# BerserkerMother/Video-Summarization

Measured on AMD Instinct MI355X. Metric: frames/sec scored (whole node), synthetic [B,T=1024,D=1024], higher is better.
Workload: dtype f32; 1 GPU; configs[2]: B=64 videos x T=1024 frames x D=1024 per GPU, scorer cfg M-A (heads 4, d_model 256, layers 4), logits + hidden state; global_batch=64, parallelism=videos sharded over 1 GPU(s), no all_gather of scores

## Files before the change

### video-summarization_amd/csrc/vs_kernels.h

```cpp
#pragma once
#include <hip/hip_runtime.h>
#include <stdint.h>

enum { VSK_STORE16 = 16, VSK_A16 = 32, VSK_F16 = 64 };
int vsk_linear(const float *A, const float *W, const float *Wf, const float *bias, float *C, int M, int N, int K,
               int relu, const float *pe, int T, int bf16, hipStream_t st);
int vsk_linear_gate(const float *A, const float *W, const float *Wf, const float *bias, const float *gate, float scale,
                    float *C, int M, int N, int K, hipStream_t st, int bf16 = 0);
int vsk_linear_relu_dropout(const float *A, const float *W, const float *Wf, const float *bias, float *C, int M, int N,
                            int K, unsigned long long seed, unsigned site, float p, hipStream_t st, int bf16 = 0);
int vsk_pack_fragments(const float *W, float *Wf, int N, int K, hipStream_t st);
int vsk_pack_fragments_f16x3(const float *W, float *Wh, int N, int K, hipStream_t st);
int vsk_qkv(const float *h, const float *Wqkv, const float *Wf, const float *bqkv, float *qkv, int B, int T, int d,
            int H, int bf16, hipStream_t st, float qscale = 1.0f);
int vsk_attention(const float *q, const float *k, const float *v, const uint8_t *mask, float *out,
                  int B, int H, int T, int dh, float scale, hipStream_t st);
int vsk_attention_packed(const float *q, const float *k, const float *v, float *out, int H, int Mtot, int dh,
                         float scale, const int *cu, const int *work, int nwork, int nw, int prec, hipStream_t st);
float vsk_attention_qscale(float scale);
int vsk_attention_bf16(const float *q, const float *k, const float *v, const uint8_t *mask, float *out,
                       int B, int H, int T, int dh, float scale, int prec, hipStream_t st);
int vsk_attention_bf16_w64(const void *q, const void *k, const void *v, const uint8_t *mask, void *out, int B, int H, int T,
                           hipStream_t st);
int vsk_attention_bf16_w64_packed(const void *q, const void *k, const void *v, void *out, int H, int Mtot, const int *cu,
                                  const int *work, int nwork, hipStream_t st);
size_t vsk_attention_probs_workspace_bytes(int B, int H, int T);
int vsk_attention_probs(const float *q, const float *k, const uint8_t *mask, float *maps, float *received, float *entropy,
                        int B, int H, int T, int dh, float scale, void *workspace, hipStream_t st);
int vsk_linear_res_ln(const float *A, const float *W, const float *Wf, const float *bias, const float *res,
                      const float *gamma, const float *beta, float *out, int M, int N, int K,
                      const float *score_w, const float *score_b, int num_classes, int sigmoid,
                      float *scores, int bf16, hipStream_t st);
int vsk_rows_res_ln(const float *a, const float *res, const float *gamma, const float *beta, float *out, int M, int d,
                    const float *score_w, const float *score_b, int num_classes, int sigmoid, float *scores,
                    hipStream_t st, void *out16 = nullptr, int dn = 0,
                    int nsplit = 0, const float *pbias = nullptr);
struct VskMatJobs {
    enum { MAX = 24 };
    const float *in[MAX];
    float *out[MAX];
    int rows[MAX], cols[MAX];
    int n;
};
int vsk_pack_fragments_batch(const VskMatJobs &jobs, hipStream_t st);
int vsk_attention_splitkv(const float *q, const float *k, const float *v, const uint8_t *mask, float *out,
                          int B, int H, int T, int dh, float scale, hipStream_t st);
int vsk_linear_parts(const float *A, const float *Wf, float *parts, int M, int N, int K, int nsplit, hipStream_t st,
                     int f16x3 = 0);
int vsk_sum_parts_pe(const float *parts, int nsplit, const float *bias, const float *pe, int T, float *out, int M, int N, hipStream_t st);
int vsk_diag_attention(const float *q, const float *k, const float *v, float *out, int B, int H, int T, float scale,
                       unsigned long long *diag, hipStream_t st);
int vsk_diag_attention_lp(const float *q, const float *k, const float *v, float *out, int B, int H, int T, float scale,
                          int prec, unsigned long long *diag, hipStream_t st);
int vsk_diag_gemm(const float *A, const float *W, const float *bias, float *C, int M, int N, int K,
                  int grid, unsigned long long *diag, hipStream_t st);
int vsk_mlp_fused(const float *H1, const float *W1, const float *b1, const float *W2, const float *b2,
                  const float *gamma, const float *beta, float *out, int M, int d,
                  const float *score_w, const float *score_b, int num_classes, int sigmoid, float *scores,
                  hipStream_t st);
bool vsk_mlp_bf16_supported(int d);
size_t vsk_mlp_bf16_image_bytes(int d);
int vsk_pack_mlp_bf16(const float *Wo, const float *W1, const float *W2, void *img, int d, hipStream_t st);
struct VskNextQkv {
    const void *img;
    const float *bqkv;
// ... 12 lines not shown
                 const float *gamma, const float *beta, float *out, int M, int d,
                 const float *score_w, const float *score_b, int num_classes, int sigmoid, float *scores,
                 const VskNextQkv *next, hipStream_t st);
int vsk_plan_packed(const int *lengths_dev, int B, int qb, int *cu, int *work, int work_cap, hipStream_t st);
int vsk_gather_rows(const float *pe, const int *cu, int B, int tmax, int d, float *rows, hipStream_t st);
enum { VSK_COPY_MAX_SEGS = 20 };
struct VskCopySegs {
    const float *src[VSK_COPY_MAX_SEGS];
    float *dst[VSK_COPY_MAX_SEGS];
    unsigned n[VSK_COPY_MAX_SEGS];
    int count;
};
int vsk_copy_segments(const VskCopySegs &segs, hipStream_t st);
int vsk_insert_cls(const float *e, const float *cls, const uint8_t *mask, float *h, uint8_t *mask1, int B, int T, int d,
                   hipStream_t st);
int vsk_skinny_max_rows();

struct VskOptions {
    int skinny_rows;
    int lp_min_rows;
    int train_lp_min_rows;
    int lp_min_rows_fused;
    int gemm_nwm2;
    int gemm_nj2;
    int attn_nw4;
    int attn_lp_simple;
    int attn_w64;
    int lp_store32;
    int lp_mlp_unfused;
    int lp_tail_unfused;
    int lp_qkv_unfused;
    int lp_tile256;
    int lp_embed_unfused;
    int mlp_fusion;
    int mlp_abl;
    int attn_w64_checked;
    int attn_legacy;
    int attn_w64_abl;
};
VskOptions &vsk_options();
int vsk_device_cus();

bool vsk_gemm16_supported(int M, int N, int K);
int vsk_gemm16(const void *A16, const void *W16, const float *bias, void *C, int M, int N, int K, int epi, int c16,
               int T, int H, int dh, float qscale, hipStream_t st);
int vsk_to_bf16(const float *src, void *dst, size_t n, hipStream_t st);
```

### video-summarization_amd/csrc/vs_kernels.hip

```cpp
#include <atomic>

#include "vs_train_device.h"
#include "vs_kernels.h"

namespace {

enum { EPI_BIAS = 0, EPI_RELU = 1, EPI_PE = 2, EPI_QKV = 3,
       EPI_GATE = 4,
       EPI_RELU_DROP = 5 };
struct EpiArgs {
    unsigned long long seed;
    unsigned site;
    float p;
    float scale;
};

__device__ __forceinline__ unsigned long long stamp() { return vs_stamp(); }

template <int EPI, int NWM = 2, int DIAG = 0, int NJ = 2, int PREC = 0, int C16 = 0, int KW = 32, int A16 = 0>
__global__ __launch_bounds__(128 * NWM, 2) void gemm_nt_128(
    const float *__restrict__ A, const float *__restrict__ W, const float *__restrict__ bias,
    float *__restrict__ C, int M, int N, int K, const float *__restrict__ pe, int T, int H, int dh,
    unsigned long long *__restrict__ diag = nullptr, EpiArgs ea = EpiArgs{0ull, 0u, 0.f, 0.f}) {
    static_assert(KW == 32 || (KW == 64 && (PREC == 1 || PREC == 3)), "64-wide k-tiles exist for the 16-bit operands only");
// ... 516 lines not shown
            if (row < M) out[(size_t)row * N + cbase + 32 * j] = y;
        }
    }
    if (score_w != nullptr) {
        for (int c = 0; c < num_classes; ++c) {
            __syncthreads();
            float wj[NB];
#pragma unroll
            for (int j = 0; j < NB; ++j) wj[j] = score_w[(size_t)c * N + cbase + 32 * j];
#pragma unroll
            for (int t = 0; t < 16; ++t) {
                float s = 0.f;
#pragma unroll
                for (int j = 0; j < NB; ++j) s += acc[j][t] * wj[j];
                part[t] = half_sum(s);
            }
            if (r == 0) {
#pragma unroll
                for (int t = 0; t < 16; ++t) red[wc * 64 + 32 * wr + acc_row(t, h)] = part[t];
            }
            __syncthreads();
            if (tid < 64) {
                const int row = m0 + tid;
                if (row < M) {
                    float s = red[tid] + red[64 + tid] + score_b[c];
                    if (sigmoid) s = 1.0f / (1.0f + expf(-s));
                    scores[(size_t)row * num_classes + c] = s;
                }
            }
        }
    }
}

template <int NT, int PREC = 0, int A16 = 0, int DIAG = 0>
__global__ __launch_bounds__(256, 2) void gemm_ln_rows(
    const float *__restrict__ A, const float *__restrict__ W, const float *__restrict__ bias,
    const float *__restrict__ res, const float *__restrict__ gamma, const float *__restrict__ beta,
    float *__restrict__ out, int M, int K,
    const float *__restrict__ score_w, const float *__restrict__ score_b, int num_classes,
    int sigmoid, float *__restrict__ scores, unsigned long long *__restrict__ diag = nullptr) {
    constexpr int BM = 128, N = 32 * NT, BK = 16, LD = BK + 4;
    constexpr int WL = (N * BK / 4 + 255) / 256;
    __shared__ __attribute__((aligned(16))) float smem[2 * (BM + N) * LD + 4 * N];
    float *gam_s = smem + 2 * (BM + N) * LD, *bet_s = gam_s + N, *sw_s = bet_s + N, *bias_s = sw_s + N;

    const int tid = threadIdx.x, lane = tid & 63, wave = tid >> 6;
    const int r = lane & 31, h = lane >> 5;
    const int ntiles = (M + BM - 1) / BM;
    const int nk = K / BK;

    constexpr float SC = PREC == 2 ? F16X3_WS : 1.0f;
    for (int i = tid; i < N; i += 256) { gam_s[i] = gamma[i]; bet_s[i] = beta[i]; bias_s[i] = bias[i] * SC; }

    const int lrow = tid >> 2, lc4 = (tid & 3) * 4;
    f32x4 pa[2], pw[WL];
    u32x2 pa16[2];
    const float *aptr[2], *wptr[WL];
    const unsigned short *aptr16[2];
#pragma unroll
    for (int i = 0; i < WL; ++i) {
        int wrow = lrow + 64 * i; wrow = wrow < N ? wrow : N - 1;
        wptr[i] = W + (size_t)wrow * K + lc4;
    }
    static_assert(PREC != 0 || N % 64 == 0, "the exact-fp32 staging map covers W without a guard");
    __amdgpu_buffer_rsrc_t ars = __builtin_amdgcn_make_buffer_rsrc(const_cast<float *>(A), 0, 0, 0x00020000);
    const __amdgpu_buffer_rsrc_t wrs = __builtin_amdgcn_make_buffer_rsrc(const_cast<float *>(W), 0, N * K * 4, 0x00020000);
    int aoff[2], woff[WL];
#pragma unroll
    for (int i = 0; i < WL; ++i) woff[i] = ((lrow + 64 * i) * K + lc4) * 4;
    auto gload = [&](int i, int kb) __attribute__((always_inline)) {
        if (i < 2) pa[i] = __builtin_bit_cast(f32x4, __builtin_amdgcn_raw_buffer_load_b128(ars, aoff[i], kb, 0));
        else pw[i - 2] = __builtin_bit_cast(f32x4, __builtin_amdgcn_raw_buffer_load_b128(wrs, woff[i - 2], kb, 0));
    };
    constexpr int LDB = 12;
    auto stage = [&](int buf) __attribute__((always_inline)) {
        float *As = smem + buf * (BM + N) * LD, *Ws = As + BM * LD;
        if constexpr (PREC == 2) {
#pragma unroll
            for (int i = 0; i < 2; ++i) {
                u32x2 hi, lo;
                split_f16x4((const float *)&pa[i], hi, lo);
                *(u32x2 *)&As[(lrow + 64 * i) * LD + lc4 / 2] = hi;
                *(u32x2 *)&As[(lrow + 64 * i) * LD + 8 + lc4 / 2] = lo;
            }
#pragma unroll
            for (int i = 0; i < WL; ++i)
                if (lrow + 64 * i < N) {
                    u32x2 hi, lo;
                    const f32x4 ws = pw[i] * F16X3_WS;
                    split_f16x4((const float *)&ws, hi, lo);
                    *(u32x2 *)&Ws[(lrow + 64 * i) * LD + lc4 / 2] = hi;
                    *(u32x2 *)&Ws[(lrow + 64 * i) * LD + 8 + lc4 / 2] = lo;
                }
        } else if constexpr (PREC == 1) {
#pragma unroll
            for (int i = 0; i < 2; ++i) {
                u32x2 u;
                if constexpr (A16 != 0) u = pa16[i];
                else { u[0] = pack_bf16(pa[i][0], pa[i][1]); u[1] = pack_bf16(pa[i][2], pa[i][3]); }
                *(u32x2 *)&As[(lrow + 64 * i) * LDB + lc4 / 2] = u;
            }
#pragma unroll
            for (int i = 0; i < WL; ++i)
                if (lrow + 64 * i < N) {
                    u32x2 u; u[0] = pack_bf16(pw[i][0], pw[i][1]); u[1] = pack_bf16(pw[i][2], pw[i][3]);
                    *(u32x2 *)&Ws[(lrow + 64 * i) * LDB + lc4 / 2] = u;
                }
        } else {
#pragma unroll
            for (int i = 0; i < 2; ++i) *(f32x4 *)&As[(lrow + 64 * i) * LD + lc4] = pa[i];
#pragma unroll
            for (int i = 0; i < WL; ++i) *(f32x4 *)&Ws[(lrow + 64 * i) * LD + lc4] = pw[i];
        }
    };

    f32x16 acc[NT];
    unsigned long long dsum[3] = {0, 0, 0}, tbegin = 0, tq = 0, ktiles = 0;
    if constexpr (DIAG != 0) tbegin = stamp();
    for (int tile = blockIdx.x; tile < ntiles; tile += gridDim.x) {
        if constexpr (DIAG != 0) tq = stamp();
        const int m0 = tile * BM;
        int row = m0 + 32 * wave + r;
        const bool row_ok = row < M;
        row = row_ok ? row : M - 1;
#pragma unroll
        for (int i = 0; i < 2; ++i) {
            int ar = m0 + lrow + 64 * i; ar = ar < M ? ar : M - 1;
            if constexpr (A16 != 0) {
                aptr16[i] = (const unsigned short *)A + (size_t)ar * K + lc4;
                pa16[i] = *(const u32x2 *)aptr16[i];
            } else if constexpr (PREC == 0) {
                aoff[i] = ((ar - m0) * K + lc4) * 4;
            } else {
                aptr[i] = A + (size_t)ar * K + lc4;
                pa[i] = *(const f32x4 *)aptr[i];
            }
        }
        if constexpr (PREC == 0) {
            ars = __builtin_amdgcn_make_buffer_rsrc(const_cast<float *>(A + (size_t)m0 * K), 0, (M - m0 < BM ? M - m0 : BM) * K * 4, 0x00020000);
#pragma unroll
            for (int i = 0; i < 2 + WL; ++i) gload(i, 0);
        } else {
#pragma unroll
            for (int i = 0; i < WL; ++i) pw[i] = *(const f32x4 *)wptr[i];
        }
        {
            const float *rp = res + (size_t)row * N + 4 * h;
#pragma unroll
            for (int j = 0; j < NT; ++j)
// ... 71 lines not shown
                int nld = 0, nwr = 0;
#pragma unroll
                for (int q = 0; q < LPS; ++q) {
                    const int il = t * LPS + q, iw = (t - WB) * LPS + q;
                    if (il < NL) { gload(il, kn * (BK * 4)); ++nld; }
                    if (t >= WB && iw < NL) {
                        float *Ad = smem + ((kt + 1) & 1) * (BM + N) * LD, *Wd = Ad + BM * LD;
                        if (iw < 2) *(f32x4 *)&Ad[(lrow + 64 * iw) * LD + lc4] = pa[iw];
                        else *(f32x4 *)&Wd[(lrow + 64 * (iw - 2)) * LD + lc4] = pw[iw - 2];
                        ++nwr;
                    }
                }
#pragma unroll
                for (int s2 = 0; s2 < 4; ++s2) acc[j] = MFMA32(fw[t % 3][s2], fa[g][s2], acc[j]);
                __builtin_amdgcn_sched_group_barrier(0x008, 1, 0);
                if (t + 2 < NS) __builtin_amdgcn_sched_group_barrier(0x100, 1, 0);
#pragma unroll
                for (int q = 0; q < LPS; ++q)
                    if (q < nld) __builtin_amdgcn_sched_group_barrier(0x020, 1, 0);
                __builtin_amdgcn_sched_group_barrier(0x008, 3, 0);
#pragma unroll
                for (int q = 0; q < LPS; ++q)
                    if (q < nwr) __builtin_amdgcn_sched_group_barrier(0x200, 1, 0);
                __builtin_amdgcn_sched_barrier(0);
            }
            if constexpr (DIAG != 0) {
                const unsigned long long tb = stamp();
                __syncthreads();
                dsum[0] += stamp() - tb;
            } else
                __syncthreads();
        }
        if constexpr (DIAG != 0) tq = stamp();

        float sum = 0.f;
#pragma unroll
        for (int j = 0; j < NT; ++j) {
            float pj = 0.f;
#pragma unroll
            for (int q = 0; q < 4; ++q) {
                const f32x4 bv = *(const f32x4 *)&bias_s[32 * j + 8 * q + 4 * h];
#pragma unroll
                for (int e = 0; e < 4; ++e) { acc[j][4 * q + e] += bv[e]; pj += acc[j][4 * q + e]; }
            }
            sum += pj;
        }
        sum = pair_sum(sum);
        const float mean = sum * (1.0f / N);
        float sq = 0.f;
#pragma unroll
        for (int j = 0; j < NT; ++j) {
            float pj = 0.f;
#pragma unroll
            for (int t = 0; t < 16; ++t) { const float c = acc[j][t] - mean; acc[j][t] = c; pj += c * c; }
            sq += pj;
        }
        sq = pair_sum(sq);
        const float rstd = 1.0f / sqrtf(sq * (1.0f / N) + 1e-5f * (SC * SC));
        float *tp = smem + wave * (32 * 36);
        const int trow = lane >> 3, tc4 = (lane & 7) * 4;
#pragma unroll
        for (int j = 0; j < NT; ++j) {
#pragma unroll
            for (int q = 0; q < 4; ++q) {
                const f32x4 gv = *(const f32x4 *)&gam_s[32 * j + 8 * q + 4 * h];
                const f32x4 bv = *(const f32x4 *)&bet_s[32 * j + 8 * q + 4 * h];
// ... 5 lines not shown
#pragma unroll
            for (int pq = 0; pq < 4; ++pq) {
                const f32x4 v = *(const f32x4 *)&tp[(trow + 8 * pq) * 36 + tc4];
                const int orow = m0 + 32 * wave + trow + 8 * pq;
                if (orow < M) *(f32x4 *)(out + (size_t)orow * N + 32 * j + tc4) = v;
            }
        }
        if (score_w != nullptr) {
            for (int c = 0; c < num_classes; ++c) {
                __syncthreads();
                for (int i = tid; i < N; i += 256) sw_s[i] = score_w[(size_t)c * N + i];
                __syncthreads();
                float dot = 0.f;
#pragma unroll
                for (int j = 0; j < NT; ++j) {
                    float pj = 0.f;
#pragma unroll
                    for (int q = 0; q < 4; ++q) {
                        const f32x4 wv = *(const f32x4 *)&sw_s[32 * j + 8 * q + 4 * h];
#pragma unroll
                        for (int e = 0; e < 4; ++e) pj += acc[j][4 * q + e] * wv[e];
                    }
                    dot += pj;
                }
                dot = pair_sum(dot);
                if (h == 0 && row_ok) {
                    float sc = dot + score_b[c];
                    if (sigmoid) sc = 1.0f / (1.0f + expf(-sc));
                    scores[(size_t)row * num_classes + c] = sc;
                }
            }
        }
        if constexpr (DIAG != 0) dsum[1] += stamp() - tq;
    }
    if constexpr (DIAG != 0) {
        if (diag != nullptr && lane == 0) {
            unsigned long long *o = diag + ((size_t)blockIdx.x * 4 + wave) * 8;
            o[0] = dsum[0]; o[1] = dsum[1]; o[2] = dsum[2]; o[3] = 0; o[4] = 0;
            o[5] = stamp() - tbegin; o[6] = ktiles; o[7] = tbegin;
        }
    }
}

#ifdef VS_WITH_DIAG
template <int ABL>
__global__ __launch_bounds__(256, 1) void mlp_fused_256(
    const float *__restrict__ H1, const float *__restrict__ W1, const float *__restrict__ b1,
    const float *__restrict__ W2, const float *__restrict__ b2, const float *__restrict__ gamma,
    const float *__restrict__ beta, float *__restrict__ out, int M,
    const float *__restrict__ score_w, const float *__restrict__ score_b, int num_classes,
    int sigmoid, float *__restrict__ scores) {
    constexpr int D = 256, HID = 1024, CH = 128, BK = 32, LD = BK + 4, NT = 8;
    constexpr int BUF = 256 * LD;
    __shared__ __attribute__((aligned(16))) float smem[2 * BUF + 4 * D];
    float *gam_s = smem + 2 * BUF, *bet_s = gam_s + D, *sw_s = bet_s + D, *bias_s = sw_s + D;

    const int tid = threadIdx.x, lane = tid & 63, wave = tid >> 6;
    const int r = lane & 31, h = lane >> 5;
    for (int i = tid; i < D; i += 256) { gam_s[i] = gamma[i]; bet_s[i] = beta[i]; bias_s[i] = b2[i]; }

    constexpr int LD1 = 68, LD2 = 36;
    const int r1 = tid >> 4, c1 = (tid & 15) * 4;
    const int r2 = tid >> 3, c2 = (tid & 7) * 4;
    f32x4 pa[8];
    auto load_w1 = [&](int c, int kt) __attribute__((always_inline)) {
        const float *p = W1 + (size_t)(CH * c + r1) * D + 64 * kt + c1;
#pragma unroll
        for (int i = 0; i < 8; ++i) pa[i] = *(const f32x4 *)(p + (size_t)16 * i * D);
    };
    auto load_w2 = [&](int c, int kt) __attribute__((always_inline)) {
        const float *p = W2 + (size_t)r2 * HID + CH * c + BK * kt + c2;
#pragma unroll
        for (int i = 0; i < 8; ++i) pa[i] = *(const f32x4 *)(p + (size_t)32 * i * HID);
    };
// ... 1236 lines not shown
        if (blocks > (M + 127) / 128) blocks = (M + 127) / 128;
#define VSK_LNR_CASE(NT_)                                                                             \
    case NT_:                                                                                         \
        hipLaunchKernelGGL((gemm_ln_rows<NT_, 0>), dim3(blocks), dim3(256), 0, st, A, W, bias, res, gamma, \
                           beta, out, M, K, score_w, score_b, num_classes, sigmoid, scores);          \
        break;
        switch (N / 32) {
            VSK_LNR_CASE(2) VSK_LNR_CASE(4) VSK_LNR_CASE(6) VSK_LNR_CASE(8)
            default: return -1;
        }
#undef VSK_LNR_CASE
        VSK_CHECK_LAUNCH();
        return 0;
    }
    const int blocks = (M + 63) / 64;
#define VSK_LN_CASE(NB_)                                                                                  \
    case NB_:                                                                                             \
        if (bf16 == 2)                                                                                    \
            hipLaunchKernelGGL((gemm_res_ln<NB_, 2>), dim3(blocks), dim3(256), 0, st, A, W, bias, res, gamma, \
                               beta, out, M, K, score_w, score_b, num_classes, sigmoid, scores);          \
        else                                                                                              \
            hipLaunchKernelGGL((gemm_res_ln<NB_, 0>), dim3(blocks), dim3(256), 0, st, A, W, bias, res, gamma, \
                               beta, out, M, K, score_w, score_b, num_classes, sigmoid, scores);          \
        break;
    switch (N / 64) {
        VSK_LN_CASE(1) VSK_LN_CASE(2) VSK_LN_CASE(3) VSK_LN_CASE(4)
        VSK_LN_CASE(5) VSK_LN_CASE(6) VSK_LN_CASE(7) VSK_LN_CASE(8)
        default: return -1;
    }
#undef VSK_LN_CASE
    VSK_CHECK_LAUNCH();
    return 0;
}
```

### video-summarization_amd/csrc/vs_scorer.cpp

```cpp
#include "vs_scorer.h"
#include "vs_inspect.h"

#include <hip/hip_runtime.h>

#include <atomic>
#include <cmath>
#include <cstdarg>
#include <cstdio>
#include <cstdlib>
#include <cstring>
#include <mutex>
#include <string>
#include <vector>

#include "vs_kernels.h"
#include "vs_train_kernels.h"
#include "vs_weights_impl.h"

namespace {

thread_local std::string g_err;

int fail(int code, const char *fmt, ...) {
    char buf[512];
// ... 54 lines not shown
        if (!on) return;
        (void)hipEventRecord(b, st);
        std::lock_guard<std::mutex> lk(g_prof_mu);
        g_prof.push_back({stage, a, b});
    }
};

int check_desc(const vs_model_desc *d) {
    if (!d) return fail(VS_ERR_INVALID, "desc is NULL");
    if (d->d_model <= 0 || d->d_model % 64 || d->d_model > 1024)
        return fail(VS_ERR_INVALID, "d_model=%d unsupported (multiple of 64, <= 1024)", d->d_model);
    if (d->num_heads <= 0 || d->d_model % d->num_heads)
        return fail(VS_ERR_INVALID, "d_model=%d not divisible by num_heads=%d", d->d_model, d->num_heads);
    const int dh = d->d_model / d->num_heads;
    if (dh != 32 && dh != 64 && dh != 128 && dh != 256)
        return fail(VS_ERR_INVALID, "head_dim=%d unsupported (32, 64, 128 or 256)", dh);
    if (d->num_layers < 1) return fail(VS_ERR_INVALID, "num_layers=%d unsupported (>= 1)", d->num_layers);
    if (d->in_features <= 0 || d->in_features % 32)
        return fail(VS_ERR_INVALID, "in_features=%d unsupported (multiple of 32)", d->in_features);
    if (d->num_classes <= 0) return fail(VS_ERR_INVALID, "num_classes=%d", d->num_classes);
    if (d->max_len < 0) return fail(VS_ERR_INVALID, "max_len=%d", d->max_len);
    return VS_OK;
}

}

namespace {
struct OptionName { const char *name; int VskOptions::*field; int dflt; };
const OptionName kOptions[] = {
    {"VS_SKINNY_ROWS", &VskOptions::skinny_rows, 16384}, {"VS_LP_MIN_ROWS", &VskOptions::lp_min_rows, 8192},
    {"VS_GEMM_NWM2", &VskOptions::gemm_nwm2, 0},         {"VS_GEMM_NJ2", &VskOptions::gemm_nj2, 0},
    {"VS_ATTN_NW4", &VskOptions::attn_nw4, 0},           {"VS_ATTN_LP_SIMPLE", &VskOptions::attn_lp_simple, 0},
    {"VS_MLP_FUSION", &VskOptions::mlp_fusion, 0},       {"VS_MLP_ABL", &VskOptions::mlp_abl, 0},
    {"VS_ATTN_LEGACY", &VskOptions::attn_legacy, 0},     {"VS_LP_STORE32", &VskOptions::lp_store32, 0},
    {"VS_LP_MLP_UNFUSED", &VskOptions::lp_mlp_unfused, 0}, {"VS_LP_TAIL_UNFUSED", &VskOptions::lp_tail_unfused, 0},
    {"VS_LP_QKV_UNFUSED", &VskOptions::lp_qkv_unfused, 0}, {"VS_LP_EMBED_UNFUSED", &VskOptions::lp_embed_unfused, 0},
    {"VS_LP_MIN_ROWS_FUSED", &VskOptions::lp_min_rows_fused, 256}, {"VS_LP_TILE256", &VskOptions::lp_tile256, 0},
    {"VS_ATTN_W64_CHECKED", &VskOptions::attn_w64_checked, 0}, {"VS_TRAIN_LP_MIN_ROWS", &VskOptions::train_lp_min_rows, 1024},
    {"VS_ATTN_W64", &VskOptions::attn_w64, 1},           {"VS_ATTN_W64_ABL", &VskOptions::attn_w64_abl, 0},
};
int option_from_env(const OptionName &o) {
    const char *e = getenv(o.name);
    if (!e) return o.dflt;
    return *e ? atoi(e) : 1;
}
}

VskOptions &vsk_options() {
    static VskOptions opts = [] {
        VskOptions o{};
        for (const auto &k : kOptions) o.*(k.field) = option_from_env(k);
        return o;
    }();
    return opts;
}

int vsk_device_cus() {
    static std::atomic<int> cus[64];
    int dev = 0;
    if (hipGetDevice(&dev) != hipSuccess) return -1;
    if (dev >= 0 && dev < 64) { const int c = cus[dev].load(std::memory_order_relaxed); if (c > 0) return c; }
    int n = 0;
    if (hipDeviceGetAttribute(&n, hipDeviceAttributeMultiprocessorCount, dev) != hipSuccess || n <= 0) return -1;
    if (dev >= 0 && dev < 64) cus[dev].store(n, std::memory_order_relaxed);
    return n;
}
// ... 268 lines not shown
    hipStream_t st = (hipStream_t)stream;
    const int d = D.d_model, H = D.num_heads, L = D.num_layers, M = B * T;
    const size_t md = align_up((size_t)M * d * sizeof(float), 256) / sizeof(float);
    float *ws = (float *)workspace;
    float *h0 = ws, *h1 = ws + md, *qkv = ws + 2 * md, *att = ws + 5 * md, *ffn = ws + 6 * md;
    const int dn = w->dn();
    const bool embedded = w->embedded();
    const float scale = 1.0f / sqrtf((float)dn);
    const int sig = (flags & VS_FLAG_SIGMOID) ? 1 : 0;
    const VskOptions &opt = vsk_options();
    const bool fused_ok = !embedded && vsk_mlp_bf16_supported(d) && (pk ? pk->prec == 1 : (flags & VS_FLAG_BF16_ATTENTION) != 0) &&
                          !opt.lp_store32 && !opt.lp_mlp_unfused && !opt.attn_lp_simple;
    const int lp_min_rows = fused_ok && opt.lp_min_rows_fused < opt.lp_min_rows ? opt.lp_min_rows_fused
                                                                               : opt.lp_min_rows;
    const int lbf = (flags & VS_FLAG_F16X3_LINEAR) ? 2 : ((flags & VS_FLAG_BF16_LINEAR) && M > lp_min_rows) ? 1 : 0;
    const bool splitk = (flags & VS_FLAG_SPLITK) && (lbf == 0 || lbf == 2) && !pk && !cls && M <= vsk_skinny_max_rows() && (d == 128 || d == 256 || d == 512);
    const int lnbf = lbf;
    {
        const int rows_min = cls ? B * Tf : M;
        const bool wide16 = lbf == 1 && d > 256;
        const unsigned fam = lbf == 1 ? (VSW_BF16 | (wide16 ? VSW_ROWS16 : 0u)) : rows_min > vsk_skinny_max_rows() ? 0u : lbf == 2 ? VSW_F16X3 : VSW_FRAGMENTS;
        vsw_order(w, stream);
        if (fam) if (int rc = vsw_ensure(w, fam, stream)) return rc;
    }
    const int aprec = pk ? pk->prec : (flags & VS_FLAG_F16X3_ATTENTION) ? 2 : (flags & VS_FLAG_BF16_ATTENTION) ? 1 : 0;
    const bool qkv16 = lbf == 1 && aprec == 1 && d <= 256 && !embedded && !vsk_options().lp_store32 && !vsk_options().attn_lp_simple;
    const bool ffn16 = lbf == 1 && d <= 256 && !embedded && !vsk_options().lp_store32;
    const bool mlp16 = lbf == 1 && !embedded && vsk_mlp_bf16_supported(d) && !vsk_options().lp_mlp_unfused && !vsk_options().lp_store32;
    const bool ring = lbf == 1 && aprec == 1 && !pk && d > 256 && !opt.lp_store32 && vsk_gemm16_supported(M, d, d);
    const size_t kv_stride = (qkv16 || ring) ? (size_t)M * d / 2 : (size_t)M * d;
    void *h16 = ffn + 2 * md;

    const bool qkv_fused = mlp16 && qkv16 && !vsk_options().lp_qkv_unfused;
    bool have_qkv = false;
    const float *pe_rows = pk ? pk->pe_rows : (w->has_pe ? w->p(w->pe) : nullptr);
    if (cls) {
        StageScope ps(VS_STAGE_EMBED, st);
        VS_LAUNCH(vsk_linear(x, w->p(w->embed_w), w->p(lbf == 2 ? w->h_embed_w : w->f_embed_w), w->p(w->embed_b), h1, B * Tf, d,
                             D.in_features, 0, pe_rows, Tf, lbf, st));
        uint8_t *mask1 = key_pad_mask ? (uint8_t *)workspace + need_core : nullptr;
        VS_LAUNCH(vsk_insert_cls(h1, cls, key_pad_mask, h0, mask1, B, Tf, d, st));
        key_pad_mask = mask1;
    } else if (lbf == 1 && w->has_b_embed && qkv_fused && L > 0 && !vsk_options().lp_embed_unfused) {
        StageScope ps(VS_STAGE_EMBED, st);
        const LayerOff &N = w->layers[0];
        const VskNextQkv nq{w->p(N.b_qkv), w->p(N.bqkv), qkv, T, H, vsk_attention_qscale(scale)};
        VS_LAUNCH(vsk_embed_bf16(x, w->p(w->b_embed), w->p(w->embed_b), pe_rows, T, h0, M, d, D.in_features, &nq, st));
        have_qkv = true;
    } else if (splitk && D.in_features % 1024 == 0) {
        StageScope ps(VS_STAGE_EMBED, st);
        VS_LAUNCH(vsk_linear_parts(x, w->p(lbf == 2 ? w->h_embed_w : w->f_embed_w), qkv, M, d, D.in_features, 8, st, lbf == 2));
        VS_LAUNCH(vsk_sum_parts_pe(qkv, 8, w->p(w->embed_b), pe_rows, T, h0, M, d, st));
    } else {
        StageScope ps(VS_STAGE_EMBED, st);
        VS_LAUNCH(vsk_linear(x, w->p(w->embed_w), w->p(lbf == 2 ? w->h_embed_w : w->f_embed_w), w->p(w->embed_b), h0, M, d, D.in_features, 0,
                             pe_rows, T, lbf, st));
    }
    if (ring && L > 0) VS_LAUNCH(vsk_to_bf16(h0, h16, (size_t)M * d, st));
    for (int l = 0; l < L; ++l) {
        const LayerOff &P = w->layers[l];
        const bool last = l == L - 1;
        if (ring) {
            const float qs = vsk_attention_qscale(scale);
            {
                StageScope ps(VS_STAGE_QKV, st);
                VS_LAUNCH(vsk_gemm16(h16, w->p(P.r_wqkv), w->p(P.bqkv), qkv, M, 3 * d, d, 3, 1, T, H, d / H, qs, st));
// ... 39 lines not shown
                const size_t rows = (size_t)B * H * T;
                VS_LAUNCH(vsk_attention_probs(qkv, qkv + (size_t)M * d, key_pad_mask, ins->maps ? ins->maps + i * rows * T : nullptr,
                                              ins->received ? ins->received + i * rows : nullptr,
                                              ins->entropy ? ins->entropy + i * rows : nullptr, B, H, T, d / H, scale, ins->workspace, st));
            }
        }
        {
            StageScope ps(VS_STAGE_ATTENTION, st);
            if (pk)
                VS_LAUNCH(vsk_attention_packed(qkv, qkv + kv_stride, qkv + 2 * kv_stride, att, H, M, d / H, scale,
                                               pk->cu, pk->work, pk->nwork, pk->nw, qkv16 ? (1 | VSK_STORE16) : pk->prec, st));
            else if (d / H == 256)
                VS_LAUNCH(vst_attention_fwd(qkv, qkv + (size_t)M * d, qkv + 2 * (size_t)M * d, key_pad_mask, att, ffn, B, H, T, 256, scale,
                                            0ull, 0u, 0.f, st, nullptr));
            else if (splitk && aprec != 1 && (d / H == 32 || d / H == 64 || d / H == 128))
                VS_LAUNCH(vsk_attention_splitkv(qkv, qkv + (size_t)M * d, qkv + 2 * (size_t)M * d, key_pad_mask, att, B, H, T, d / H, scale, st));
            else if (aprec)
                VS_LAUNCH(vsk_attention_bf16(qkv, qkv + kv_stride, qkv + 2 * kv_stride, key_pad_mask, att,
                                             B, H, T, d / H, scale, qkv16 ? (1 | VSK_STORE16) : aprec, st));
            else
                VS_LAUNCH(vsk_attention(qkv, qkv + (size_t)M * d, qkv + 2 * (size_t)M * d, key_pad_mask, att, B, H,
                                        T, d / H, scale, st));
        }
        float *dst = (last && hidden) ? hidden : h0;
        if (mlp16 && qkv16 && !vsk_options().lp_tail_unfused) {
            StageScope ps(VS_STAGE_FC2_LN, st);
            VS_LAUNCH(vsk_mlp_bf16(h0, att, w->p(P.bo), w->p(P.ln1g), w->p(P.ln1b), w->p(P.b_mlp), w->p(P.b1), w->p(P.b2),
                                   w->p(P.ln2g), w->p(P.ln2b), dst, M, d, last ? w->p(w->final_w) : nullptr,
                                   last ? w->p(w->final_b) : nullptr, D.num_classes, sig, last ? scores : nullptr, next, st));
            have_qkv = next != nullptr;
            continue;
        }
        have_qkv = false;
        const bool split_ln = d > 256 || embedded;
        {
            StageScope ps(VS_STAGE_OUTPROJ_LN, st);
            if (splitk && d >= 256) {
                const int so = 2;
                VS_LAUNCH(vsk_linear_parts(att, w->p(lbf == 2 ? P.h_wo : P.f_wo), qkv, M, d, d, so, st, lbf == 2));
                VS_LAUNCH(vsk_rows_res_ln(qkv, h0, w->p(P.ln1g), w->p(P.ln1b), h1, M, d, nullptr, nullptr, 0, 0, nullptr, st, nullptr, dn,
                                          so, w->p(P.bo)));
            } else if (split_ln) {
                VS_LAUNCH(vsk_linear(att, w->p(P.wo), w->p(lnbf == 2 ? P.h_wo : P.f_wo), w->p(P.bo), qkv, M, d, d, 0, nullptr, 1, lnbf, st));
                VS_LAUNCH(vsk_rows_res_ln(qkv, h0, w->p(P.ln1g), w->p(P.ln1b), h1, M, d, nullptr, nullptr, 0, 0, nullptr, st, nullptr, dn));
            } else
            VS_LAUNCH(vsk_linear_res_ln(att, w->p(P.wo), w->p(lnbf == 2 ? P.h_wo : P.f_wo), w->p(P.bo), h0, w->p(P.ln1g), w->p(P.ln1b), h1, M, d, d,
                                        nullptr, nullptr, 0, 0, nullptr, qkv16 ? (1 | VSK_STORE16) : lnbf, st));
        }
#ifdef VS_WITH_DIAG
        const bool fused = d == 256 && vsk_options().mlp_fusion != 0 && M > vsk_skinny_max_rows() && !lbf;
        if (fused) {
            StageScope ps(VS_STAGE_FC2_LN, st);
            VS_LAUNCH(vsk_mlp_fused(h1, w->p(P.w1), w->p(P.b1), w->p(P.w2), w->p(P.b2), w->p(P.ln2g), w->p(P.ln2b), dst, M, d,
                                    last ? w->p(w->final_w) : nullptr, last ? w->p(w->final_b) : nullptr,
                                    D.num_classes, sig, last ? scores : nullptr, st));
            continue;
        }
#endif
        if (mlp16) {
            StageScope ps(VS_STAGE_FC2_LN, st);
            VS_LAUNCH(vsk_mlp_bf16(h1, nullptr, nullptr, nullptr, nullptr, w->p(P.b_mlp), w->p(P.b1), w->p(P.b2), w->p(P.ln2g), w->p(P.ln2b), dst, M, d,
                                   last ? w->p(w->final_w) : nullptr, last ? w->p(w->final_b) : nullptr,
                                   D.num_classes, sig, last ? scores : nullptr, next, st));
            have_qkv = next != nullptr;
            continue;
        }
// ... 407 lines not shown
```

Measured before the change: 11.77 million frames/s.

## Fuse out-proj+LN with FC1 and FC2+LN with next-layer QKV for fp32 d=256

Adds two persistent kernels for the exact fp32 path at d_model 256. The first runs the attention out-projection with residual and LayerNorm, then feeds the normalized tile from registers straight into the FC1 GEMM with ReLU. The second runs FC2 with residual and LayerNorm, then computes the next layer's QKV projection and writes it in head-major layout. This removes separate launches and the global round trips of the normalized activations. In exchange the kernels grow more complex, use more shared memory and registers, and stream the full second weight matrix through every row tile, which may limit occupancy.

```diff
diff --git a/video-summarization_amd/csrc/vs_kernels.h b/video-summarization_amd/csrc/vs_kernels.h
--- a/video-summarization_amd/csrc/vs_kernels.h
+++ b/video-summarization_amd/csrc/vs_kernels.h
@@ -31,6 +31,11 @@
                       const float *gamma, const float *beta, float *out, int M, int N, int K,
                       const float *score_w, const float *score_b, int num_classes, int sigmoid,
                       float *scores, int bf16, hipStream_t st);
+bool vsk_layer_fused_supported(int M, int d);
+int vsk_outproj_ln_fc1(const float *att, const float *Wo, const float *bo, const float *res, const float *gamma, const float *beta,
+                       float *h1, const float *W1, const float *b1, float *hidden, int M, int d, hipStream_t st);
+int vsk_fc2_ln_qkv(const float *hidden, const float *W2, const float *b2, const float *res, const float *gamma, const float *beta,
+                   float *out, const float *Wqkv, const float *bqkv, float *qkv, int B, int T, int d, int H, hipStream_t st);
 int vsk_rows_res_ln(const float *a, const float *res, const float *gamma, const float *beta, float *out, int M, int d,
                     const float *score_w, const float *score_b, int num_classes, int sigmoid, float *scores,
                     hipStream_t st, void *out16 = nullptr, int dn = 0,
@@ -109,6 +114,7 @@
     int lp_qkv_unfused;
     int lp_tile256;
     int lp_embed_unfused;
+    int exact_unfused;
     int mlp_fusion;
     int mlp_abl;
     int attn_w64_checked;
diff --git a/video-summarization_amd/csrc/vs_kernels.hip b/video-summarization_amd/csrc/vs_kernels.hip
--- a/video-summarization_amd/csrc/vs_kernels.hip
+++ b/video-summarization_amd/csrc/vs_kernels.hip
@@ -572,17 +572,26 @@
     }
 }
 
-template <int NT, int PREC = 0, int A16 = 0, int DIAG = 0>
-__global__ __launch_bounds__(256, 2) void gemm_ln_rows(
+struct LnTail {
+    const float *W2, *b2;
+    float *C2;
+    int T, H, dhs;
+};
+
+template <int NT, int PREC, int A16, int DIAG, int TAIL>
+__device__ __forceinline__ void ln_rows_tiles(
     const float *__restrict__ A, const float *__restrict__ W, const float *__restrict__ bias,
     const float *__restrict__ res, const float *__restrict__ gamma, const float *__restrict__ beta,
     float *__restrict__ out, int M, int K,
     const float *__restrict__ score_w, const float *__restrict__ score_b, int num_classes,
-    int sigmoid, float *__restrict__ scores, unsigned long long *__restrict__ diag = nullptr) {
+    int sigmoid, float *__restrict__ scores, unsigned long long *__restrict__ diag, const LnTail tl) {
+    static_assert(TAIL == 0 || (NT == 8 && PREC == 0 && DIAG == 0), "the register-fed tail exists for exact fp32 at d_model 256");
     constexpr int BM = 128, N = 32 * NT, BK = 16, LD = BK + 4;
     constexpr int WL = (N * BK / 4 + 255) / 256;
-    __shared__ __attribute__((aligned(16))) float smem[2 * (BM + N) * LD + 4 * N];
+    constexpr int TN2 = TAIL == 2 ? 3 * N : 4 * N;
+    __shared__ __attribute__((aligned(16))) float smem[2 * (BM + N) * LD + 4 * N + (TAIL != 0 ? TN2 : 0)];
     float *gam_s = smem + 2 * (BM + N) * LD, *bet_s = gam_s + N, *sw_s = bet_s + N, *bias_s = sw_s + N;
+    float *bias2_s = bias_s + N;
 
     const int tid = threadIdx.x, lane = tid & 63, wave = tid >> 6;
     const int r = lane & 31, h = lane >> 5;
@@ -591,6 +600,8 @@
 
     constexpr float SC = PREC == 2 ? F16X3_WS : 1.0f;
     for (int i = tid; i < N; i += 256) { gam_s[i] = gamma[i]; bet_s[i] = beta[i]; bias_s[i] = bias[i] * SC; }
+    if constexpr (TAIL != 0)
+        for (int i = tid; i < TN2; i += 256) bias2_s[i] = tl.b2[i];
 
     const int lrow = tid >> 2, lc4 = (tid & 3) * 4;
     f32x4 pa[2], pw[WL];
@@ -655,6 +666,56 @@
     };
 
     f32x16 acc[NT];
+
+    constexpr int TCH = 128, TNC = TN2 / TCH, TWB = 4 * 32 * 36, TBUF = TCH * 36;
+    static_assert(TAIL == 0 || TWB + 2 * TBUF <= 2 * (BM + N) * LD, "corners and weight tiles fit the staging area");
+    const int r2 = tid >> 3, c2 = (tid & 7) * 4;
+    const __amdgpu_buffer_rsrc_t wrs2 = __builtin_amdgcn_make_buffer_rsrc(const_cast<float *>(tl.W2), 0, TN2 * N * 4, 0x00020000);
+    const int woff2 = (r2 * N + c2) * 4;
+    f32x4 pw2[4];
+    f32x16 U[4];
+    auto tail_soff = [&](int c, int kt) __attribute__((always_inline)) { return (TCH * c * N + 32 * kt) * 4; };
+    auto tail_load = [&](int i, int soff) __attribute__((always_inline)) {
+        pw2[i] = __builtin_bit_cast(f32x4, __builtin_amdgcn_raw_buffer_load_b128(wrs2, woff2, soff + 32 * i * N * 4, 0));
+    };
+    auto tail_stage = [&](int buf) __attribute__((always_inline)) {
+#pragma unroll
+        for (int i = 0; i < 4; ++i) *(f32x4 *)&smem[TWB + buf * TBUF + (r2 + 32 * i) * 36 + c2] = pw2[i];
+    };
+    auto bias_mfma = [&](int c) __attribute__((always_inline)) {
+        const f32x16 zero = {0.f, 0.f, 0.f, 0.f, 0.f, 0.f, 0.f, 0.f, 0.f, 0.f, 0.f, 0.f, 0.f, 0.f, 0.f, 0.f};
+#pragma unroll
+        for (int jj = 0; jj < 4; ++jj) {
+            const float bv = bias2_s[TCH * c + 32 * jj + r];
+            U[jj] = MFMA32(h == 0 ? bv : 0.f, 1.0f, zero);
+        }
+    };
+    auto tail_step = [&](auto ktc, int nsoff) __attribute__((always_inline)) {
+        constexpr int kt = decltype(ktc)::value;
+        const float *wp = smem + TWB + (kt & 1) * TBUF + r * 36 + 4 * h;
+        float *wd = smem + TWB + ((kt + 1) & 1) * TBUF + r2 * 36 + c2;
+        f32x4 fw[3];
+        fw[0] = *(const f32x4 *)wp;
+        fw[1] = *(const f32x4 *)(wp + 32 * 36);
+        __builtin_amdgcn_sched_barrier(0);
+#pragma unroll
+        for (int t = 0; t < 16; ++t) {
+            const int g = t / 4, jj = t % 4;
+            if (t + 2 < 16) fw[(t + 2) % 3] = *(const f32x4 *)(wp + 32 * ((t + 2) % 4) * 36 + 8 * ((t + 2) / 4));
+            if (t < 4) tail_load(t, nsoff);
+            if (t >= 12) *(f32x4 *)(wd + 32 * (t - 12) * 36) = pw2[t - 12];
+#pragma unroll
+            for (int s2 = 0; s2 < 4; ++s2) U[jj] = MFMA32(fw[t % 3][s2], acc[kt][4 * g + s2], U[jj]);
+            __builtin_amdgcn_sched_group_barrier(0x008, 1, 0);
+            if (t + 2 < 16) __builtin_amdgcn_sched_group_barrier(0x100, 1, 0);
+            if (t < 4) __builtin_amdgcn_sched_group_barrier(0x020, 1, 0);
+            __builtin_amdgcn_sched_group_barrier(0x008, 3, 0);
+            if (t >= 12) __builtin_amdgcn_sched_group_barrier(0x200, 1, 0);
+            __builtin_amdgcn_sched_barrier(0);
+        }
+        __syncthreads();
+    };
+
     unsigned long long dsum[3] = {0, 0, 0}, tbegin = 0, tq = 0, ktiles = 0;
     if constexpr (DIAG != 0) tbegin = stamp();
     for (int tile = blockIdx.x; tile < ntiles; tile += gridDim.x) {
@@ -792,6 +853,10 @@
                 __syncthreads();
         }
         if constexpr (DIAG != 0) tq = stamp();
+        if constexpr (TAIL != 0) {
+#pragma unroll
+            for (int i = 0; i < 4; ++i) tail_load(i, tail_soff(0, 0));
+        }
 
         float sum = 0.f;
 #pragma unroll
@@ -863,6 +928,61 @@
             }
         }
         if constexpr (DIAG != 0) dsum[1] += stamp() - tq;
+        if constexpr (TAIL != 0) {
+            tail_stage(0);
+            int rowoff[4];
+            __amdgpu_buffer_rsrc_t crs;
+            if constexpr (TAIL == 1) {
+                crs = __builtin_amdgcn_make_buffer_rsrc(tl.C2 + (size_t)m0 * TN2, 0, (M - m0 < BM ? M - m0 : BM) * TN2 * 4, 0x00020000);
+#pragma unroll
+                for (int p = 0; p < 4; ++p) rowoff[p] = ((32 * wave + trow + 8 * p) * TN2 + tc4) * 4;
+            } else {
+                crs = __builtin_amdgcn_make_buffer_rsrc(tl.C2, 0, 0, 0x00020000);
+#pragma unroll
+                for (int p = 0; p < 4; ++p) {
+                    const int orow = m0 + 32 * wave + trow + 8 * p;
+                    const int bb = orow / tl.T, tt = orow - bb * tl.T;
+                    rowoff[p] = orow < M ? (((bb * tl.H * tl.T + tt) << tl.dhs) + tc4) * 4 : (int)0x80000000;
+                }
+            }
+            bias_mfma(0);
+            __syncthreads();
+            for (int c = 0; c < TNC; ++c) {
+                const int cn = c + 1 < TNC ? c + 1 : c;
+                static_for<8>([&](auto ktc) __attribute__((always_inline)) {
+                    constexpr int kt = decltype(ktc)::value;
+                    tail_step(ktc, kt < 7 ? tail_soff(c, kt + 1) : tail_soff(cn, 0));
+                });
+                if constexpr (TAIL == 2) {
+                    const int which = c >> 1;
+                    crs = __builtin_amdgcn_make_buffer_rsrc(tl.C2 + (size_t)which * M * N, 0, M * N * 4, 0x00020000);
+                }
+#pragma unroll
+                for (int jj = 0; jj < 4; ++jj) {
+                    __builtin_amdgcn_sched_barrier(0);
+#pragma unroll
+                    for (int q = 0; q < 4; ++q) {
+                        f32x4 v;
+#pragma unroll
+                        for (int e = 0; e < 4; ++e) v[e] = TAIL == 1 ? relu1(U[jj][4 * q + e]) : U[jj][4 * q + e];
+                        *(f32x4 *)&tp[r * 36 + 8 * q + 4 * h] = v;
+                    }
+                    int soff;
+                    if constexpr (TAIL == 1) soff = (TCH * c + 32 * jj) * 4;
+                    else {
+                        const int cc = (TCH * c + 32 * jj) & (N - 1), head = cc >> tl.dhs, e0 = cc - (head << tl.dhs);
+                        soff = (((head * tl.T) << tl.dhs) + e0) * 4;
+                    }
+#pragma unroll
+                    for (int p = 0; p < 4; ++p) {
+                        const f32x4 v = *(const f32x4 *)&tp[(trow + 8 * p) * 36 + tc4];
+                        __builtin_amdgcn_raw_buffer_store_b128(__builtin_bit_cast(u32x4, v), crs, rowoff[p], soff, 0);
+                    }
+                }
+                __builtin_amdgcn_sched_barrier(0);
+                bias_mfma(cn);
+            }
+        }
     }
     if constexpr (DIAG != 0) {
         if (diag != nullptr && lane == 0) {
@@ -871,6 +991,33 @@
             o[5] = stamp() - tbegin; o[6] = ktiles; o[7] = tbegin;
         }
     }
+}
+
+template <int NT, int PREC = 0, int A16 = 0, int DIAG = 0>
+__global__ __launch_bounds__(256, 2) void gemm_ln_rows(
+    const float *__restrict__ A, const float *__restrict__ W, const float *__restrict__ bias,
+    const float *__restrict__ res, const float *__restrict__ gamma, const float *__restrict__ beta,
+    float *__restrict__ out, int M, int K,
+    const float *__restrict__ score_w, const float *__restrict__ score_b, int num_classes,
+    int sigmoid, float *__restrict__ scores, unsigned long long *__restrict__ diag = nullptr) {
+    ln_rows_tiles<NT, PREC, A16, DIAG, 0>(A, W, bias, res, gamma, beta, out, M, K, score_w, score_b, num_classes, sigmoid, scores, diag,
+                                          LnTail{nullptr, nullptr, nullptr, 0, 0, 0});
+}
+
+__global__ __launch_bounds__(256, 2) void layer_outproj_ln_fc1(
+    const float *__restrict__ A, const float *__restrict__ W, const float *__restrict__ bias,
+    const float *__restrict__ res, const float *__restrict__ gamma, const float *__restrict__ beta,
+    float *__restrict__ out, int M, int K, const float *__restrict__ W1, const float *__restrict__ b1, float *__restrict__ hidden) {
+    ln_rows_tiles<8, 0, 0, 0, 1>(A, W, bias, res, gamma, beta, out, M, K, nullptr, nullptr, 0, 0, nullptr, nullptr,
+                                 LnTail{W1, b1, hidden, 0, 0, 0});
+}
+__global__ __launch_bounds__(256, 2) void layer_fc2_ln_qkv(
+    const float *__restrict__ A, const float *__restrict__ W, const float *__restrict__ bias,
+    const float *__restrict__ res, const float *__restrict__ gamma, const float *__restrict__ beta,
+    float *__restrict__ out, int M, int K, const float *__restrict__ Wqkv, const float *__restrict__ bqkv, float *__restrict__ qkv,
+    int T, int H, int dhs) {
+    ln_rows_tiles<8, 0, 0, 0, 2>(A, W, bias, res, gamma, beta, out, M, K, nullptr, nullptr, 0, 0, nullptr, nullptr,
+                                 LnTail{Wqkv, bqkv, qkv, T, H, dhs});
 }
 
 #ifdef VS_WITH_DIAG
@@ -2173,3 +2320,30 @@
     VSK_CHECK_LAUNCH();
     return 0;
 }
+
+bool vsk_layer_fused_supported(int M, int d) { return d == 256 && M > skinny_max_rows() && M <= (1 << 20); }
+
+int vsk_outproj_ln_fc1(const float *att, const float *Wo, const float *bo, const float *res, const float *gamma, const float *beta,
+                       float *h1, const float *W1, const float *b1, float *hidden, int M, int d, hipStream_t st) {
+    if (!vsk_layer_fused_supported(M, d)) return -1;
+    int blocks = persistent_blocks((M + 127) / 128);
+    if (blocks < 0) return (int)hipErrorInvalidDevice;
+    if (blocks > (M + 127) / 128) blocks = (M + 127) / 128;
+    hipLaunchKernelGGL(layer_outproj_ln_fc1, dim3(blocks), dim3(256), 0, st, att, Wo, bo, res, gamma, beta, h1, M, d, W1, b1, hidden);
+    VSK_CHECK_LAUNCH();
+    return 0;
+}
+
+int vsk_fc2_ln_qkv(const float *hidden, const float *W2, const float *b2, const float *res, const float *gamma, const float *beta,
+                   float *out, const float *Wqkv, const float *bqkv, float *qkv, int B, int T, int d, int H, hipStream_t st) {
+    const int M = B * T;
+    if (!vsk_layer_fused_supported(M, d) || H <= 0 || d % H || (d / H) % 32) return -1;
+    int dhs = 5;
+    while ((1 << dhs) < d / H) ++dhs;
+    int blocks = persistent_blocks((M + 127) / 128);
+    if (blocks < 0) return (int)hipErrorInvalidDevice;
+    if (blocks > (M + 127) / 128) blocks = (M + 127) / 128;
+    hipLaunchKernelGGL(layer_fc2_ln_qkv, dim3(blocks), dim3(256), 0, st, hidden, W2, b2, res, gamma, beta, out, M, 4 * d, Wqkv, bqkv, qkv, T, H, dhs);
+    VSK_CHECK_LAUNCH();
+    return 0;
+}
diff --git a/video-summarization_amd/csrc/vs_scorer.cpp b/video-summarization_amd/csrc/vs_scorer.cpp
--- a/video-summarization_amd/csrc/vs_scorer.cpp
+++ b/video-summarization_amd/csrc/vs_scorer.cpp
@@ -110,6 +110,7 @@
     {"VS_GEMM_NWM2", &VskOptions::gemm_nwm2, 0},         {"VS_GEMM_NJ2", &VskOptions::gemm_nj2, 0},
     {"VS_ATTN_NW4", &VskOptions::attn_nw4, 0},           {"VS_ATTN_LP_SIMPLE", &VskOptions::attn_lp_simple, 0},
     {"VS_MLP_FUSION", &VskOptions::mlp_fusion, 0},       {"VS_MLP_ABL", &VskOptions::mlp_abl, 0},
+    {"VS_EXACT_UNFUSED", &VskOptions::exact_unfused, 0},
     {"VS_ATTN_LEGACY", &VskOptions::attn_legacy, 0},     {"VS_LP_STORE32", &VskOptions::lp_store32, 0},
     {"VS_LP_MLP_UNFUSED", &VskOptions::lp_mlp_unfused, 0}, {"VS_LP_TAIL_UNFUSED", &VskOptions::lp_tail_unfused, 0},
     {"VS_LP_QKV_UNFUSED", &VskOptions::lp_qkv_unfused, 0}, {"VS_LP_EMBED_UNFUSED", &VskOptions::lp_embed_unfused, 0},
@@ -444,6 +445,8 @@
     void *h16 = ffn + 2 * md;
 
     const bool qkv_fused = mlp16 && qkv16 && !vsk_options().lp_qkv_unfused;
+    const bool exact_fused = lbf == 0 && aprec == 0 && !embedded && !splitk && !opt.exact_unfused && vsk_layer_fused_supported(M, d) &&
+                             d % H == 0 && (d / H) % 32 == 0;
     bool have_qkv = false;
     const float *pe_rows = pk ? pk->pe_rows : (w->has_pe ? w->p(w->pe) : nullptr);
     if (cls) {
@@ -549,6 +552,23 @@
             continue;
         }
         have_qkv = false;
+        if (exact_fused) {
+            {
+                StageScope ps(VS_STAGE_FC1, st);
+                VS_LAUNCH(vsk_outproj_ln_fc1(att, w->p(P.wo), w->p(P.bo), h0, w->p(P.ln1g), w->p(P.ln1b), h1, w->p(P.w1), w->p(P.b1), ffn, M, d, st));
+            }
+            StageScope ps(VS_STAGE_FC2_LN, st);
+            if (last) {
+                VS_LAUNCH(vsk_linear_res_ln(ffn, w->p(P.w2), w->p(P.f_w2), w->p(P.b2), h1, w->p(P.ln2g), w->p(P.ln2b), dst, M, d, 4 * d,
+                                            w->p(w->final_w), w->p(w->final_b), D.num_classes, sig, scores, 0, st));
+            } else {
+                const LayerOff &N = w->layers[l + 1];
+                VS_LAUNCH(vsk_fc2_ln_qkv(ffn, w->p(P.w2), w->p(P.b2), h1, w->p(P.ln2g), w->p(P.ln2b), dst, w->p(N.wqkv), w->p(N.bqkv), qkv,
+                                         B, T, d, H, st));
+                have_qkv = true;
+            }
+            continue;
+        }
         const bool split_ln = d > 256 || embedded;
         {
             StageScope ps(VS_STAGE_OUTPROJ_LN, st);
```

Measured after the change: 12.04 million frames/s, median of 6. 1.02x the previous value.
